# sandialabs/implicit-sph

Measured on AMD Instinct MI355X. Metric: pressure-Poisson solves/sec (3D TGV, 1M particles per GPU, GMRES(50)+block-Jacobi ILU(0), tol 1e-8), higher is better.
Workload: dtype f64; 1 GPU; 3D Taylor-Green vortex, 100^3 particles per GPU, Wendland cut=2h (BASELINE configs[1]), state after one Lagrangian step (mode=advect); rows_per_gpu=1000000, global_rows=1000000, nnz_per_gpu=103845090, solver=FGMRES(50) DGKS tol 1e-8, right prec, precond=bjacobi-ilu0, atom_order=lexicographic, library_row_order=bricks, parallelism=domain bricks 1x1x1, RCCL halo + all-reduce, restarts=1, converged=1

## Files before the change

### implicit-sph_amd/csrc/core.hpp

```cpp
#pragma once
#include "common.hpp"
#include "order.hpp"
#include "sell.hpp"

namespace isph { struct HostStager; }

struct isph_neigh_layout {
  const void *nptr = nullptr;
  const int *nidx = nullptr, *colmap = nullptr;
  const void *order = nullptr;
  int n = -1, is_sorted = 0;
  isph::DevBuf<long long> off;
  isph::DevBuf<int> idx, len, sorted;
  void release() { off.release(); idx.release(); len.release(); sorted.release(); nptr = nullptr; nidx = colmap = nullptr; order = nullptr; n = -1; is_sorted = 0; }
};

struct isph_neigh_map {
  const int *rowsrc = nullptr, *idmap = nullptr, *colmap_key = nullptr;
  const int *colkey = nullptr;
  const void *order = nullptr;
};

struct isph_table_cache {
  int ntypes = -1, kernel = -1, dim = -1;
  std::vector<int> kind;
  std::vector<double> h, cutsq;
  isph::DevBuf<int> dkind;
  isph::DevBuf<double> dh, dcutsq, dhinv, dknorm, dkdnorm;
  void release() { dkind.release(); dh.release(); dcutsq.release(); dhinv.release(); dknorm.release(); dkdnorm.release(); ntypes = -1; }
};

struct isph_ctx {
  int device = 0;
  hipStream_t stream = nullptr;
  bool own_stream = false;
  int rank = 0, nranks = 1;
  ncclComm_t comm = nullptr;
  isph_host_transport host_tr = {nullptr, nullptr, nullptr};
  double *hsend = nullptr, *hrecv = nullptr;
  size_t hsend_cap = 0, hrecv_cap = 0;
  bool profile = false;
  int stat_reorth = 0;
  isph::DevBuf<double> partial;
  isph::DevBuf<double> dscal;
  double *hscal = nullptr;
  size_t hscal_cap = 0;
  isph::DevBuf<double> V, Z, wv, tv, rv, pv, nvec, xext, sendbuf, bdev, xdev;
  isph::DevBuf<float> V32;
  isph::DevBuf<double> vcur;
  isph::DevBuf<double> bint, xint;
  isph::DevBuf<int> imask, imask2;
  std::vector<hipEvent_t> ev;
  std::vector<int> ev_class;
  size_t ev_used = 0;
  std::vector<hipEvent_t> hev;
  size_t hev_used = 0;
  hipEvent_t ev0 = nullptr, ev1 = nullptr;
  hipEvent_t ev_fetch = nullptr;
  std::vector<hipEvent_t> ev_ls;
  hipStream_t comm_stream = nullptr;
  hipEvent_t ev_pack = nullptr, ev_halo = nullptr;
  isph::DevBuf<double> xghost;
  isph::HostStager *stager = nullptr;
  bool neigh_hold = false;
  bool pattern_hold = false;
  isph_neigh_layout neigh_cache[2];
  isph_table_cache tables;
  int ordering = 1;
  isph::OrderBox box;
  isph_neigh_map nmap;
  isph::RowOrderPtr held_order;
  const void *held_key[2] = {nullptr, nullptr};
};

namespace isph {
enum ProfClass { PROF_SPMV = 0, PROF_PREC_APPLY, PROF_MULTI_DOT, PROF_MULTI_AXPY_DOT, PROF_MULTI_AXPY_NORM, PROF_ILU_EXTRACT,
                 PROF_ILU_SCHEDULE, PROF_ILU_FACTOR, PROF_NCLASS };
struct ProfScope {
  isph_ctx *c;
  size_t slot = (size_t)-1;
  ProfScope(isph_ctx *ctx, int cls, hipStream_t st = nullptr) : c(ctx) {
    if (!c || !c->profile || (st && st != c->stream)) return;
    if (c->ev_used + 2 > c->ev.size()) {
      hipEvent_t a = nullptr, b = nullptr;
      if (hipEventCreate(&a) != hipSuccess || hipEventCreate(&b) != hipSuccess) return;
      c->ev.push_back(a); c->ev.push_back(b);
      c->ev_class.push_back(cls);
    }
    slot = c->ev_used;
    c->ev_class[slot / 2] = cls;
    c->ev_used += 2;
    (void)hipEventRecord(c->ev[slot], c->stream);
  }
  ~ProfScope() { end(); }
  void end() {
    if (slot != (size_t)-1) (void)hipEventRecord(c->ev[slot + 1], c->stream);
    slot = (size_t)-1;
  }
};
}

struct isph_halo {
  int npeers = 0;
  std::vector<int> peer, send_ptr, recv_ptr;
  isph::DevBuf<int> send_idx;
  int nsend = 0, nrecv = 0;
  isph::DevBuf<int> list_int, list_bnd;
  int n_int = 0, n_bnd = 0;
};

struct isph_pb_rows;
namespace isph { void pb_rows_destroy(isph_pb_rows *R); }

struct isph_mat {
  isph::Sell S;
  isph_halo halo;
  isph::RowOrderPtr order;
  bool local = false;
  bool aux = false;
  isph_pb_rows *pb = nullptr;
  isph::DevBuf<unsigned> emap;
  long long n_updates = 0;
};
```

### implicit-sph_amd/csrc/gmres_host.hpp

```cpp
#pragma once
#include <algorithm>
#include <cmath>
#include <vector>

namespace isph {

struct GmresCycle {
  int m = 0, j = 0;
  std::vector<double> H, cs, sn, g, y;
  double beta = 0.0, scale = 1.0;

  void reset(int m_) {
    m = m_; j = 0;
    H.assign((size_t)(m + 1) * (size_t)m, 0.0);
    cs.assign((size_t)m, 0.0); sn.assign((size_t)m, 0.0); g.assign((size_t)m + 1, 0.0); y.assign((size_t)m, 0.0);
  }
  void start() {
    std::fill(g.begin(), g.end(), 0.0);
    g[0] = beta;
    j = 0;
  }
  double *column() { return &H[(size_t)j * (size_t)(m + 1)]; }
  double push() {
    double *h = column();
    for (int k = 0; k < j; ++k) {
      const double a = cs[k] * h[k] + sn[k] * h[k + 1];
      h[k + 1] = -sn[k] * h[k] + cs[k] * h[k + 1];
      h[k] = a;
    }
    const double a = h[j], bb = h[j + 1], rr = std::hypot(a, bb);
    cs[j] = rr == 0.0 ? 1.0 : a / rr;
    sn[j] = rr == 0.0 ? 0.0 : bb / rr;
    h[j] = rr;
    h[j + 1] = 0.0;
    g[j + 1] = -sn[j] * g[j];
    g[j] = cs[j] * g[j];
    ++j;
    return std::fabs(g[j]);
  }
  const double *solve() {
    for (int k = j - 1; k >= 0; --k) {
      double s = g[k];
      for (int l = k + 1; l < j; ++l) s -= H[(size_t)l * (size_t)(m + 1) + k] * y[l];
      y[k] = s / H[(size_t)k * (size_t)(m + 1) + k];
    }
    return y.data();
  }
};

template <typename Info>
inline bool gmres_after_update(bool f32, Info &inf, int max_iters, int max_restarts) {
  if (f32 && inf.converged) return true;
  if (inf.converged || inf.iters >= max_iters || inf.restarts >= max_restarts) return false;
  ++inf.restarts;
  return true;
}

template <typename Info>
inline bool gmres_after_residual(bool f32, Info &inf, int max_iters, int max_restarts, double beta, double scale, double tol) {
  if (f32 && inf.converged) {
    if (beta / scale <= tol) return false;
    inf.converged = 0;
    if (inf.iters >= max_iters || inf.restarts >= max_restarts) return false;
    ++inf.restarts;
    ++inf.residual_restarts;
  }
  if (beta == 0.0) { inf.converged = 1; return false; }
  return true;
}

}
```

### implicit-sph_amd/csrc/krylov.hpp

```cpp
#pragma once
#include "common.hpp"

namespace isph {

constexpr int kDotBatch = 16;

template <typename BT> struct BasisVec;
template <> struct BasisVec<double> {
  typedef double2 pair;
  typedef double *__restrict__ out;
};
struct BasisOut32 {
  float *col;
  double *cur;
};
template <> struct BasisVec<float> {
  typedef float2 pair;
  typedef BasisOut32 out;
};
__device__ __forceinline__ bool basis_out_set(const double *o) { return o != nullptr; }
__device__ __forceinline__ bool basis_out_set(const BasisOut32 &o) { return o.col != nullptr; }
__device__ __forceinline__ void basis_put(double *o, long long i, double v) { o[i] = v; }
__device__ __forceinline__ void basis_put(const BasisOut32 &o, long long i, double v) {
  const float r = static_cast<float>(v);
// ... 62 lines not shown
                                                      double *__restrict__ partial) {
  __shared__ double sred[kDotBatch + 1][4];
  const int wave = threadIdx.x >> 6, lane = threadIdx.x & 63;
  const long long stride = (long long)gridDim.x * kBlock;
  const long long i0 = (long long)blockIdx.x * kBlock + threadIdx.x;
  for (int k0 = 0; k0 < nk || k0 == 0; k0 += kDotBatch) {
    const int nb = min(kDotBatch, nk - k0);
    const bool last = k0 + kDotBatch >= nk;
    double acc[kDotBatch];
#pragma unroll
    for (int u = 0; u < kDotBatch; ++u) acc[u] = 0.0;
    double ww = 0.0;
    const BT *__restrict__ vb = V + (long long)k0 * ld;
    long long i = i0;
    if (ROWS == 2) {
      for (; i + stride < n; i += 2 * stride) {
        const double wa = w[i], wb = w[i + stride];
        if (last) ww = fma(wb, wb, fma(wa, wa, ww));
        double va[kDotBatch], vc[kDotBatch];
#pragma unroll
        for (int u = 0; u < kDotBatch; ++u)
          if (u < nb) { va[u] = (double)vb[(long long)u * ld + i]; vc[u] = (double)vb[(long long)u * ld + i + stride]; }
#pragma unroll
        for (int u = 0; u < kDotBatch; ++u)
          if (u < nb) acc[u] = fma(vc[u], wb, fma(va[u], wa, acc[u]));
      }
    }
    for (; i < n; i += stride) {
      const double wi = w[i];
      if (last) ww = fma(wi, wi, ww);
#pragma unroll
      for (int u = 0; u < kDotBatch; ++u)
        if (u < nb) acc[u] = fma((double)vb[(long long)u * ld + i], wi, acc[u]);
    }
#pragma unroll
    for (int u = 0; u < kDotBatch; ++u) {
      if (u < nb) {
        const double s = wave_sum(acc[u]);
        if (lane == 0) sred[u][wave] = s;
      }
    }
    if (last) {
      ww = wave_sum(ww);
      if (lane == 0) sred[kDotBatch][wave] = ww;
    }
    __syncthreads();
    if (threadIdx.x < nb)
      partial[(long long)(k0 + threadIdx.x) * gridDim.x + blockIdx.x] =
          (sred[threadIdx.x][0] + sred[threadIdx.x][1]) + (sred[threadIdx.x][2] + sred[threadIdx.x][3]);
    if (last && threadIdx.x == 0)
      partial[(long long)nk * gridDim.x + blockIdx.x] =
          (sred[kDotBatch][0] + sred[kDotBatch][1]) + (sred[kDotBatch][2] + sred[kDotBatch][3]);
    __syncthreads();
    if (last) break;
  }
}

__global__ __launch_bounds__(kBlock) void k_reduce_partials(int nk, int nblk, const double *__restrict__ partial,
                                                            double *__restrict__ out,
                                                            const double *__restrict__ flag = nullptr) {
  __shared__ double sw[4];
  const int k = blockIdx.x;
  if (k >= nk) return;
  if (flag && *flag == 0.0) {
    if (threadIdx.x == 0) out[k] = 0.0;
    return;
  }
  const double *__restrict__ p = partial + (long long)k * nblk;
  double s0 = 0.0, s1 = 0.0, s2 = 0.0, s3 = 0.0;
  int b = threadIdx.x;
  for (; b + 3 * kBlock < nblk; b += 4 * kBlock) {
    s0 += p[b];
    s1 += p[b + kBlock];
    s2 += p[b + 2 * kBlock];
    s3 += p[b + 3 * kBlock];
  }
  for (; b < nblk; b += kBlock) s0 += p[b];
  double s = wave_sum((s0 + s1) + (s2 + s3));
  if ((threadIdx.x & 63) == 0) sw[threadIdx.x >> 6] = s;
  __syncthreads();
  if (threadIdx.x == 0) out[k] = (sw[0] + sw[1]) + (sw[2] + sw[3]);
}

template <typename BT>
__global__ __launch_bounds__(kBlock) void k_multi_axpy_norm(int n, int nk, const BT *__restrict__ V, long long ld,
                                                            const double *__restrict__ c, double *__restrict__ w,
                                                            double *__restrict__ partial,
                                                            const double *__restrict__ dec_old = nullptr,
                                                            const double *__restrict__ dec_dn = nullptr, int dec_force = 0,
                                                            double *__restrict__ dec_out = nullptr,
                                                            typename BasisVec<BT>::out vnext = {}) {
  __shared__ double sw[4];
  __shared__ double sdec[2];
  const bool next = basis_out_set(vnext);
  bool second = true;
  double wfinal2 = 1.0;
  if (dec_old) {
    if (threadIdx.x == 0) {
      double old2 = *dec_old;
      if (dec_dn) old2 = fmax(old2 - dec_dn[0] * dec_dn[0], 0.0);
      const double ww_new = c[nk];
      const bool sec = dec_force || sqrt(ww_new) < M_SQRT1_2 * sqrt(old2);
      double s2 = 0.0;
      for (int k = 0; k < nk; ++k) s2 += c[k] * c[k];
      sdec[0] = sec ? 1.0 : 0.0;
      sdec[1] = sec ? fmax(ww_new - s2, 0.0) : ww_new;
      if (blockIdx.x == 0) { dec_out[0] = sdec[0]; dec_out[1] = sdec[1]; }
    }
    __syncthreads();
    second = sdec[0] != 0.0;
    wfinal2 = sdec[1];
  }
  if (!second && !next) return;
  double a = 1.0;
  if (next) a *= 1.0 / sqrt(wfinal2);
  double ww = 0.0;
  for (long long i = (long long)blockIdx.x * blockDim.x + threadIdx.x; i < n; i += (long long)gridDim.x * blockDim.x) {
    double s = w[i];
    if (second) {
      for (int k = 0; k < nk; ++k) s = fma(-c[k], (double)V[(long long)k * ld + i], s);
      w[i] = s;
    }
    if (next) basis_put(vnext, i, a * s);
    ww = fma(s, s, ww);
  }
  ww = wave_sum(ww);
  if ((threadIdx.x & 63) == 0) sw[threadIdx.x >> 6] = ww;
  __syncthreads();
  if (threadIdx.x == 0) partial[blockIdx.x] = (sw[0] + sw[1]) + (sw[2] + sw[3]);
}

template <int NK, typename BT = double>
__global__ __launch_bounds__(kBlock) void k_multi_axpy_dot(int n, int nk, const BT *__restrict__ V, long long ld,
                                                           const double *__restrict__ c, double *__restrict__ w,
                                                           double *__restrict__ partial) {
  __shared__ double sred[NK + 1][4];
  __shared__ double sc[NK];
  const int wave = threadIdx.x >> 6, lane = threadIdx.x & 63;
  if (threadIdx.x < NK) sc[threadIdx.x] = threadIdx.x < nk ? c[threadIdx.x] : 0.0;
  __syncthreads();
  double acc[NK];
#pragma unroll
  for (int u = 0; u < NK; ++u) acc[u] = 0.0;
  double ww = 0.0;
  const long long stride = (long long)gridDim.x * kBlock;
  if constexpr (sizeof(BT) == 8) {
    for (long long i = (long long)blockIdx.x * kBlock + threadIdx.x; i < n; i += stride) {
      double v[NK];
#pragma unroll
      for (int u = 0; u < NK; ++u) v[u] = u < nk ? V[(long long)u * ld + i] : 0.0;
      double s = w[i];
#pragma unroll
      for (int u = 0; u < NK; ++u) s = fma(-sc[u], v[u], s);
      w[i] = s;
      ww = fma(s, s, ww);
#pragma unroll
      for (int u = 0; u < NK; ++u) acc[u] = fma(v[u], s, acc[u]);
    }
  } else {
    typedef typename BasisVec<BT>::pair pair;
    const long long np = n >> 1;
    double2 *__restrict__ w2 = reinterpret_cast<double2 *>(w);
    for (long long p = (long long)blockIdx.x * kBlock + threadIdx.x; p < np; p += stride) {
      pair v[NK];
#pragma unroll
      for (int u = 0; u < NK; ++u) {
        if (u < nk) v[u] = reinterpret_cast<const pair *>(V + (long long)u * ld)[p];
        else v[u].x = v[u].y = 0;
      }
      double2 s = w2[p];
#pragma unroll
      for (int u = 0; u < NK; ++u) {
        s.x = fma(-sc[u], (double)v[u].x, s.x);
        s.y = fma(-sc[u], (double)v[u].y, s.y);
      }
      w2[p] = s;
      ww = fma(s.y, s.y, fma(s.x, s.x, ww));
#pragma unroll
      for (int u = 0; u < NK; ++u) asm volatile("" : "+v"(v[u].x), "+v"(v[u].y));
#pragma unroll
      for (int u = 0; u < NK; ++u) acc[u] = fma((double)v[u].y, s.y, fma((double)v[u].x, s.x, acc[u]));
    }
    if ((n & 1) && blockIdx.x == 0 && threadIdx.x == 0) {
      const long long i = n - 1;
      double s = w[i];
#pragma unroll
      for (int u = 0; u < NK; ++u)
        if (u < nk) s = fma(-sc[u], (double)V[(long long)u * ld + i], s);
      w[i] = s;
      ww = fma(s, s, ww);
#pragma unroll
      for (int u = 0; u < NK; ++u)
        if (u < nk) acc[u] = fma((double)V[(long long)u * ld + i], s, acc[u]);
    }
  }
#pragma unroll
  for (int u = 0; u < NK; ++u) {
    if (u < nk) {
      const double r = wave_sum(acc[u]);
      if (lane == 0) sred[u][wave] = r;
    }
  }
  ww = wave_sum(ww);
  if (lane == 0) sred[NK][wave] = ww;
// ... 108 lines not shown
```

### implicit-sph_amd/csrc/solver.hpp

```cpp
#pragma once
#include <cmath>
#include <type_traits>

#include "comm.hpp"
#include "core.hpp"
#include "gmres_host.hpp"
#include "krylov.hpp"

namespace isph {

inline int prec_apply_dev(isph_ctx *ctx, const isph_prec *M, const double *r, double *z);
inline int prec_apply_multi_dev(isph_ctx *ctx, const isph_prec *M, int K, const double *const *rs, double *const *zs);

inline int allreduce_inplace(isph_ctx *ctx, double *d, int count) {
  return comm_allreduce(ctx, d, count,  0, ctx->stream);
}

enum { SC_DOT = 0 , SC_Y = 64 , SC_MISC = 128, SC_COUNT = 160 };

constexpr int kMaxLockstep = 4;

inline int ensure_scalars(isph_ctx *ctx) {
  ISPH_CHECK(ctx->dscal.reserve(SC_COUNT * kMaxLockstep));
  ISPH_CHECK(ctx->partial.reserve((size_t)kMaxRedBlocks * 66));
  if (ctx->hscal_cap < (size_t)SC_COUNT * kMaxLockstep) {
    if (ctx->hscal) (void)hipHostFree(ctx->hscal);
    ISPH_CHECK_HIP(hipHostMalloc((void **)&ctx->hscal, (size_t)SC_COUNT * kMaxLockstep * sizeof(double)));
    ctx->hscal_cap = (size_t)SC_COUNT * kMaxLockstep;
  }
  return ISPH_SUCCESS;
}

inline int fetch_scalars(isph_ctx *ctx, int first, int count) {
  ISPH_CHECK_HIP(hipMemcpyAsync(ctx->hscal + first, ctx->dscal.p + first, sizeof(double) * (size_t)count,
                                hipMemcpyDeviceToHost, ctx->stream));
  ISPH_CHECK_HIP(hipStreamSynchronize(ctx->stream));
  return ISPH_SUCCESS;
}

__global__ void k_gather(int n, const int *__restrict__ idx, const double *__restrict__ x, double *__restrict__ out) {
  for (int i = blockIdx.x * blockDim.x + threadIdx.x; i < n; i += gridDim.x * blockDim.x) out[i] = x[idx[i]];
}
__global__ void k_gather_widen(int n, const int *__restrict__ idx, const float *__restrict__ x, double *__restrict__ out) {
  for (int i = blockIdx.x * blockDim.x + threadIdx.x; i < n; i += gridDim.x * blockDim.x) out[i] = (double)x[idx[i]];
}
inline void halo_pack(isph_ctx *ctx, const isph_halo &H, const double *x) {
  hipLaunchKernelGGL(k_gather, dim3(stream_grid(H.nsend)), dim3(kBlock), 0, ctx->stream, H.nsend, H.send_idx.p, x,
                     ctx->sendbuf.p);
}
inline void halo_pack(isph_ctx *ctx, const isph_halo &H, const float *x) {
  hipLaunchKernelGGL(k_gather_widen, dim3(stream_grid(H.nsend)), dim3(kBlock), 0, ctx->stream, H.nsend, H.send_idx.p, x,
                     ctx->sendbuf.p);
}

template <class XT>
inline int halo_begin(isph_ctx *ctx, const isph_mat *A, const XT *x, hipEvent_t *hev = nullptr) {
  ISPH_REQUIRE(comm_active(ctx) && ctx->comm_stream,
               "a matrix with a halo needs a context made by isph_ctx_create_dist or isph_ctx_create_hostcomm");
  const Sell &S = A->S;
  const isph_halo &H = A->halo;
  ISPH_REQUIRE(H.nrecv == S.ncol - S.nrow, "matrix has ghost columns but no matching halo plan");
  ISPH_REQUIRE(H.n_int + H.n_bnd == S.nslices, "halo plan without the interior/boundary slice lists");
  ISPH_CHECK(ctx->xghost.reserve((size_t)(H.nrecv > 0 ? H.nrecv : 1)));
  ISPH_CHECK(ctx->sendbuf.reserve((size_t)(H.nsend > 0 ? H.nsend : 1)));
  if (H.nsend > 0) halo_pack(ctx, H, x);
  ISPH_CHECK_HIP(hipEventRecord(ctx->ev_pack, ctx->stream));
  if (hev) ISPH_CHECK_HIP(hipEventRecord(hev[0], ctx->stream));
  ISPH_CHECK_HIP(hipStreamWaitEvent(ctx->comm_stream, ctx->ev_pack, 0));
  ISPH_CHECK(comm_exchange(ctx, H, ctx->sendbuf.p, ctx->xghost.p, 1, false, ctx->comm_stream));
  ISPH_CHECK_HIP(hipEventRecord(ctx->ev_halo, ctx->comm_stream));
  if (hev) ISPH_CHECK_HIP(hipEventRecord(hev[1], ctx->comm_stream));
  return ISPH_SUCCESS;
}

inline bool sell_cols16(isph_ctx *ctx, const Sell &S) {
  if (S.c16_state != 0) return S.c16_state > 0;
  S.c16_state = -1;
  if (S.nslices == 0 || S.stored == 0) return false;
  DevTmp<int> flag;
  if (flag.reserve(1) != ISPH_SUCCESS || S.col16.reserve((size_t)S.stored) != ISPH_SUCCESS ||
      S.wtab.reserve((size_t)S.nslices * 64) != ISPH_SUCCESS) { flag.release(); return false; }
  int h = 0;
  if (hipMemsetAsync(flag.p, 0, sizeof(int), ctx->stream) == hipSuccess) {
    hipLaunchKernelGGL(k_sell_compress_cols, dim3((S.nslices + 3) / 4), dim3(kBlock), 0, ctx->stream, 0, S.nslices,
                       (const long long *)S.slice_off.p, (const int *)S.col.p, S.col16.p, S.wtab.p, flag.p);
    if (hipMemcpyAsync(&h, flag.p, sizeof(int), hipMemcpyDeviceToHost, ctx->stream) == hipSuccess &&
        hipStreamSynchronize(ctx->stream) == hipSuccess && hipGetLastError() == hipSuccess && h == 0)
      S.c16_state = 1;
  }
  flag.release();
  if (S.c16_state < 0) { S.col16.release(); S.wtab.release(); }
  return S.c16_state > 0;
}

template <bool DOT, bool LIST, bool GHOST>
inline void spmv_launch(isph_ctx *ctx, const Sell &S, bool c16, int nsl, const int *list, const double *x, const double *xg,
                        double *y, const double *nvec, const double *badd = nullptr, double alpha = 1.0,
                        const float *val32 = nullptr) {
  if (nsl <= 0) return;
  int nbp = 0;
  const int grid = spmv_grid(nsl, &nbp);
  double *part = DOT ? ctx->partial.p : nullptr;
  if (val32 && c16)
    hipLaunchKernelGGL((k_sell_spmv16<8, false, LIST, GHOST, float>), dim3(grid), dim3(kBlock), 0, ctx->stream, S.nrow, nsl, nbp,
                       S.slice_off.p, S.col16.p, S.wtab.p, val32, x, y, nvec, part, list, xg, badd, alpha);
  else if (val32)
    hipLaunchKernelGGL((k_sell_spmv<8, false, true, LIST, GHOST, float>), dim3(grid), dim3(kBlock), 0, ctx->stream, S.nrow, nsl, nbp,
                       S.slice_off.p, S.col.p, val32, x, y, nvec, part, list, xg, badd, alpha);
  else if (c16)
    hipLaunchKernelGGL((k_sell_spmv16<8, DOT, LIST, GHOST>), dim3(grid), dim3(kBlock), 0, ctx->stream, S.nrow, nsl, nbp,
// ... 125 lines not shown
    if (c16) {
      if (K == 2) ISPH_SPMM_AXPB(true, 2, S.col16.p, S.wtab.p);
      else if (K == 3) ISPH_SPMM_AXPB(true, 3, S.col16.p, S.wtab.p);
      else ISPH_SPMM_AXPB(true, 4, S.col16.p, S.wtab.p);
    } else {
      if (K == 2) ISPH_SPMM_AXPB(false, 2, S.col.p, nullptr);
      else if (K == 3) ISPH_SPMM_AXPB(false, 3, S.col.p, nullptr);
      else ISPH_SPMM_AXPB(false, 4, S.col.p, nullptr);
    }
  }
#undef ISPH_SPMM_AXPB
  prof.end();
  ISPH_CHECK_HIP(hipGetLastError());
  return ISPH_SUCCESS;
}

struct LinOp {
  isph_ctx *ctx;
  const isph_mat *A;
  const isph_prec *M;
  const double *nvec;
  int n;
  int dim = 1, nloc = 0;
  const isph_mat *const *blk = nullptr;
  double *tmp = nullptr;
  int apply(const double *x, double *y) const {
    if (blk) {
      for (int i = 0; i < dim; ++i) {
        double *yi = y + (size_t)i * nloc;
        bool first = true;
        for (int j = 0; j < dim; ++j) {
          const isph_mat *B = blk[i * dim + j];
          if (!B) continue;
          ISPH_CHECK(spmv_dev(ctx, B, x + (size_t)j * nloc, first ? yi : tmp, nullptr));
          if (!first)
            hipLaunchKernelGGL(k_axpy_dev, dim3(stream_grid(nloc)), dim3(kBlock), 0, ctx->stream, nloc, 1.0,
                               (const double *)nullptr, (const double *)tmp, yi);
          first = false;
        }
        if (first) ISPH_CHECK_HIP(hipMemsetAsync(yi, 0, sizeof(double) * (size_t)nloc, ctx->stream));
      }
      return ISPH_SUCCESS;
    }
    ISPH_CHECK(spmv_dev(ctx, A, x, y, nvec));
    if (nvec)
      hipLaunchKernelGGL(k_axpy_dev, dim3(stream_grid(n)), dim3(kBlock), 0, ctx->stream, n, -1.0,
                         ctx->dscal.p + SC_MISC, nvec, y);
    return ISPH_SUCCESS;
  }
  int prec(const double *r, double *z) const {
    if (!M) {
      ISPH_CHECK_HIP(hipMemcpyAsync(z, r, sizeof(double) * (size_t)n, hipMemcpyDeviceToDevice, ctx->stream));
      return ISPH_SUCCESS;
    }
    if (blk) {
      const double *rs[4];
      double *zs[4];
      for (int i = 0; i < dim && i < 4; ++i) { rs[i] = r + (size_t)i * nloc; zs[i] = z + (size_t)i * nloc; }
      return prec_apply_multi_dev(ctx, M, dim, rs, zs);
    }
    return prec_apply_dev(ctx, M, r, z);
  }
};

inline int dot_dev(isph_ctx *ctx, int n, const double *a, const double *b, const double *c, const double *d, int slot) {
  const int g = stream_grid(n);
  hipLaunchKernelGGL(k_dot2, dim3(g), dim3(kBlock), 0, ctx->stream, n, a, b, c, d, ctx->partial.p);
  hipLaunchKernelGGL(k_reduce_partials, dim3(2), dim3(kBlock), 0, ctx->stream, 2, g, ctx->partial.p, ctx->dscal.p + slot);
  return allreduce_inplace(ctx, ctx->dscal.p + slot, 2);
}

inline int norm_host(isph_ctx *ctx, int n, const double *v, double *out) {
  ISPH_CHECK(dot_dev(ctx, n, v, v, nullptr, nullptr, SC_MISC + 4));
  ISPH_CHECK(fetch_scalars(ctx, SC_MISC + 4, 1));
  *out = std::sqrt(ctx->hscal[SC_MISC + 4]);
  return ISPH_SUCCESS;
}

inline int residual_norm(isph_ctx *ctx, int n, const double *b, double *w, double *out) {
  hipLaunchKernelGGL(k_residual, dim3(stream_grid(n)), dim3(kBlock), 0, ctx->stream, n, b, w);
  return norm_host(ctx, n, w, out);
}

inline int upload_y(isph_ctx *ctx, GmresCycle &c, int mb = 0) {
  std::copy_n(c.solve(), c.j, ctx->hscal + mb + SC_Y);
  ISPH_CHECK_HIP(hipMemcpyAsync(ctx->dscal.p + mb + SC_Y, ctx->hscal + mb + SC_Y, sizeof(double) * (size_t)c.j, hipMemcpyHostToDevice, ctx->stream));
  return ISPH_SUCCESS;
}

inline int project_dev(isph_ctx *ctx, int n, const double *nvec, double *v) {
  ISPH_CHECK(dot_dev(ctx, n, v, nvec, nullptr, nullptr, SC_MISC + 2));
  hipLaunchKernelGGL(k_axpy_dev, dim3(stream_grid(n)), dim3(kBlock), 0, ctx->stream, n, -1.0, ctx->dscal.p + SC_MISC + 2,
                     nvec, v);
  return ISPH_SUCCESS;
}

inline int cgs_pass(isph_ctx *ctx, int n, int nk, const double *V, long long ld, double *w) {
  int g = stream_grid(n);
  if (g > 1024) g = 1024;
  ISPH_CHECK(ctx->partial.reserve((size_t)(nk + 2) * kMaxRedBlocks > (size_t)kMaxRedBlocks * 66 ? (size_t)(nk + 2) * kMaxRedBlocks : (size_t)kMaxRedBlocks * 66));
  hipLaunchKernelGGL((k_multi_dot<1>), dim3(g), dim3(kBlock), 0, ctx->stream, n, nk, V, ld, w, ctx->partial.p);
  hipLaunchKernelGGL(k_reduce_partials, dim3(nk + 1), dim3(kBlock), 0, ctx->stream, nk + 1, g, ctx->partial.p,
                     ctx->dscal.p + SC_DOT);
  ISPH_CHECK(allreduce_inplace(ctx, ctx->dscal.p + SC_DOT, nk + 1));
  const int g2 = stream_grid(n);
  hipLaunchKernelGGL(k_multi_axpy_norm<double>, dim3(g2), dim3(kBlock), 0, ctx->stream, n, nk, V, ld, ctx->dscal.p + SC_DOT, w,
                     ctx->partial.p);
  hipLaunchKernelGGL(k_reduce_partials, dim3(1), dim3(kBlock), 0, ctx->stream, 1, g2, ctx->partial.p,
                     ctx->dscal.p + SC_DOT + nk + 1);
  ISPH_CHECK(allreduce_inplace(ctx, ctx->dscal.p + SC_DOT + nk + 1, 1));
  ISPH_CHECK_HIP(hipGetLastError());
  return fetch_scalars(ctx, SC_DOT, nk + 2);
}

enum { SC_ORTHO = SC_MISC + 20 };
template <typename BT>
inline int ortho_enqueue(isph_ctx *ctx, int n, int nk, const BT *V, long long ld, double *w, int ortho,
                         typename BasisVec<BT>::out vnext, bool deflate = false, int mb = 0) {
  int g = stream_grid(n);
  if (g > 1024) g = 1024;
  ISPH_CHECK(ctx->partial.reserve((size_t)kMaxRedBlocks * 66));
  hipStream_t st = ctx->stream;
  if (sizeof(BT) == 4)
    ISPH_REQUIRE((reinterpret_cast<uintptr_t>(w) & 15) == 0 && (reinterpret_cast<uintptr_t>(V) & 7) == 0 && ld % 2 == 0,
                 "basis_bits = 32: the Krylov vectors must be 16-byte aligned");
  double *dh1 = ctx->dscal.p + mb + SC_DOT, *dh2 = ctx->dscal.p + mb + SC_Y, *dor = ctx->dscal.p + mb + SC_ORTHO;
  constexpr int dot_grid = 512;
  if (g > dot_grid) g = dot_grid;
  {
    ProfScope prof(ctx, PROF_MULTI_DOT);
    if ((reinterpret_cast<uintptr_t>(w) & 15) == 0 && (reinterpret_cast<uintptr_t>(V) & 15) == 0)
      hipLaunchKernelGGL(k_multi_dot_v2<BT>, dim3(g), dim3(kBlock), 0, st, n, nk, V, ld, w, ctx->partial.p);
    else
      hipLaunchKernelGGL((k_multi_dot<2, BT>), dim3(g), dim3(kBlock), 0, st, n, nk, V, ld, w, ctx->partial.p);
  }
  hipLaunchKernelGGL(k_reduce_partials, dim3(nk + 1), dim3(kBlock), 0, st, nk + 1, g, ctx->partial.p, dh1,
                     (const double *)nullptr);
  ISPH_CHECK(allreduce_inplace(ctx, dh1, nk + 1));
  {
    ProfScope prof(ctx, PROF_MULTI_AXPY_DOT);
    if (nk <= 16)
      hipLaunchKernelGGL((k_multi_axpy_dot<16, BT>), dim3(g), dim3(kBlock), 0, st, n, nk, V, ld, dh1, w, ctx->partial.p);
    else if (nk <= 32)
      hipLaunchKernelGGL((k_multi_axpy_dot<32, BT>), dim3(g), dim3(kBlock), 0, st, n, nk, V, ld, dh1, w, ctx->partial.p);
    else if (nk <= 48)
      hipLaunchKernelGGL((k_multi_axpy_dot<48, BT>), dim3(g), dim3(kBlock), 0, st, n, nk, V, ld, dh1, w, ctx->partial.p);
    else
      hipLaunchKernelGGL((k_multi_axpy_dot<64, BT>), dim3(g), dim3(kBlock), 0, st, n, nk, V, ld, dh1, w, ctx->partial.p);
  }
  hipLaunchKernelGGL(k_reduce_partials, dim3(nk + 1), dim3(kBlock), 0, st, nk + 1, g, ctx->partial.p, dh2,
                     (const double *)nullptr);
  ISPH_CHECK(allreduce_inplace(ctx, dh2, nk + 1));
  const int g2 = stream_grid(n);
  {
    ProfScope prof(ctx, PROF_MULTI_AXPY_NORM);
    hipLaunchKernelGGL(k_multi_axpy_norm<BT>, dim3(g2), dim3(kBlock), 0, st, n, nk, V, ld, (const double *)dh2, w, ctx->partial.p,
                       (const double *)(dh1 + nk), deflate ? (const double *)dh1 : (const double *)nullptr, ortho == 1 ? 1 : 0,
                       dor, vnext);
  }
  ISPH_CHECK_HIP(hipGetLastError());
  return ISPH_SUCCESS;
}

inline void ortho_collect(isph_ctx *ctx, int nk, double *h, double *wnorm, int mb = 0) {
  const double *hs = ctx->hscal + mb;
  const bool second = hs[SC_ORTHO] != 0.0;
  if (second) ++ctx->stat_reorth;
  for (int k = 0; k < nk; ++k) h[k] = hs[SC_DOT + k] + (second ? hs[SC_Y + k] : 0.0);
  *wnorm = std::sqrt(hs[SC_ORTHO + 1]);
}

inline int orthogonalize(isph_ctx *ctx, int n, int j, const double *V, long long ld, double *w, double *h, int ortho,
                         double *wnorm) {
  const int nk = j + 1;
  for (int k = 0; k < nk; ++k) h[k] = 0.0;
  if (ortho == 2) {
    double nn = 0.0;
    for (int pass = 0; pass < 2; ++pass)
      for (int k = 0; k < nk; ++k) {
        ISPH_CHECK(cgs_pass(ctx, n, 1, V + (long long)k * ld, ld, w));
        h[k] += ctx->hscal[SC_DOT];
        nn = ctx->hscal[SC_DOT + 2];
      }
    *wnorm = std::sqrt(nn);
    return ISPH_SUCCESS;
  }
  ISPH_CHECK(ortho_enqueue<double>(ctx, n, nk, V, ld, w, ortho, nullptr));
  ISPH_CHECK(fetch_scalars(ctx, 0, SC_COUNT));
  ortho_collect(ctx, nk, h, wnorm);
  return ISPH_SUCCESS;
}

inline int basis_bits_of(const isph_solver_params *prm, int *bits) {
  *bits = prm->basis_bits == 0 ? 64 : prm->basis_bits;
  ISPH_REQUIRE(*bits == 64 || *bits == 32, "basis_bits must be 64 (0 means the same) or 32");
  return ISPH_SUCCESS;
}

template <typename BT>
inline int gmres_t(const LinOp &op, const double *b, double *x, const isph_solver_params *prm, isph_solve_info *info) {
  constexpr bool f32 = std::is_same<BT, float>::value;
  isph_ctx *ctx = op.ctx;
  const int n = op.n, m = prm->num_blocks;
  ISPH_REQUIRE(m >= 1 && m <= 62, "Num Blocks must be in [1,62]");
  const long long ld = ((long long)n + 63) / 64 * 64;
  const bool deflate = !f32 && op.nvec != nullptr && !op.blk && prm->ortho != 2;
  if (f32) {
    ctx->V.release();
    ISPH_CHECK(ctx->V32.reserve((size_t)ld * (size_t)(m + 1)));
    ISPH_CHECK(ctx->vcur.reserve((size_t)ld));
  } else {
    ctx->V32.release();
    ctx->vcur.release();
    ISPH_CHECK(ctx->V.reserve((size_t)ld * (size_t)(m + 2)));
  }
  if (prm->flexible) ISPH_CHECK(ctx->Z.reserve((size_t)ld * (size_t)m));
  ISPH_CHECK(ctx->wv.reserve((size_t)ld));
  ISPH_CHECK(ctx->tv.reserve((size_t)ld));
  BT *Vall, *V;
  if constexpr (f32) Vall = V = ctx->V32.p;
  else { Vall = ctx->V.p; V = ctx->V.p + (deflate ? ld : 0); }
  double *Z = ctx->Z.p, *w = ctx->wv.p, *t = ctx->tv.p, *vcur = ctx->vcur.p;
  auto column = [&](int col) -> typename BasisVec<BT>::out {
    if constexpr (f32) return BasisOut32{V + (long long)col * ld, vcur};
    else return V + (long long)col * ld;
  };
  if constexpr (!f32)
    if (deflate)
    ISPH_CHECK_HIP(hipMemcpyAsync(Vall, op.nvec, sizeof(double) * (size_t)n, hipMemcpyDeviceToDevice, ctx->stream));
  GmresCycle c;
  c.reset(m);
  const int sg = stream_grid(n);
  hipStream_t st = ctx->stream;

  ISPH_CHECK(op.apply(x, w));
  ISPH_CHECK(residual_norm(ctx, n, b, w, &c.beta));
  c.scale = c.beta == 0.0 ? 1.0 : c.beta;
  info->iters = 0;
  info->restarts = 0;
  info->residual_restarts = 0;
  info->converged = 0;
  info->rel_res_implicit = c.beta / c.scale;
  if (c.beta / c.scale <= prm->tol) info->converged = 1;

  while (!info->converged && info->iters < prm->max_iters) {
    hipLaunchKernelGGL(k_scale_copy<BT>, dim3(sg), dim3(kBlock), 0, st, n, (const double *)w, column(0), 1.0 / c.beta, (const double *)nullptr, 0);
    c.start();
    auto enqueue_op = [&](int col) -> int {
      const double *zj, *vj;
      if constexpr (f32) vj = vcur;
      else vj = V + (long long)col * ld;
      if (prm->flexible) {
        ISPH_CHECK(op.prec(vj, Z + (long long)col * ld));
        zj = Z + (long long)col * ld;
      } else {
        ISPH_CHECK(op.prec(vj, t));
        zj = t;
      }
      return deflate ? spmv_dev(ctx, op.A, zj, w, nullptr) : op.apply(zj, w);
    };
    bool op_queued = false;
    while (c.j < m) {
      const int j = c.j;
      if (!op_queued) ISPH_CHECK(enqueue_op(j));
      op_queued = false;
      double *h = c.column();
      double wn = 0.0;
      if (prm->ortho == 2) {
        if constexpr (!f32) {
          ISPH_CHECK(orthogonalize(ctx, n, j, V, ld, w, h, prm->ortho, &wn));
          if (wn != 0.0)
            hipLaunchKernelGGL(k_scale_copy<double>, dim3(sg), dim3(kBlock), 0, st, n, w, V + (long long)(j + 1) * ld, 1.0 / wn,
                               (const double *)nullptr, 0);
        }
      } else {
        const int nkt = j + 1 + (deflate ? 1 : 0);
        ISPH_CHECK(ortho_enqueue<BT>(ctx, n, nkt, Vall, ld, w, prm->ortho, column(j + 1), deflate));
        ISPH_CHECK_HIP(hipMemcpyAsync(ctx->hscal, ctx->dscal.p, sizeof(double) * SC_COUNT, hipMemcpyDeviceToHost, st));
        ISPH_CHECK_HIP(hipEventRecord(ctx->ev_fetch, st));
        if (j + 1 < m && info->iters + 1 < prm->max_iters) {
          ISPH_CHECK(enqueue_op(j + 1));
          op_queued = true;
        }
        ISPH_CHECK_HIP(hipEventSynchronize(ctx->ev_fetch));
        if (deflate) {
          double hh[66];
          ortho_collect(ctx, nkt, hh, &wn);
          for (int k = 0; k <= j; ++k) h[k] = hh[k + 1];
        } else {
          ortho_collect(ctx, nkt, h, &wn);
        }
      }
      h[j + 1] = wn;
      ++info->iters;
      info->rel_res_implicit = c.push() / c.scale;
      if (prm->verbose && ctx->rank == 0 && info->iters % 10 == 0)
        printf(">> isph::gmres iter %d  rel res %.3e\n", info->iters, info->rel_res_implicit);
      if (info->rel_res_implicit <= prm->tol) { info->converged = 1; break; }
      if (info->iters >= prm->max_iters) break;
    }
    const int j = c.j;
    ISPH_CHECK(upload_y(ctx, c));
    if (prm->flexible) {
      hipLaunchKernelGGL(k_multi_axpy<double>, dim3(sg), dim3(kBlock), 0, st, n, j, Z, ld, ctx->dscal.p + SC_Y, x);
    } else {
      hipLaunchKernelGGL(k_fill, dim3(sg), dim3(kBlock), 0, st, n, w, 0.0);
      hipLaunchKernelGGL(k_multi_axpy<BT>, dim3(sg), dim3(kBlock), 0, st, n, j, (const BT *)V, ld, (const double *)(ctx->dscal.p + SC_Y), w);
      ISPH_CHECK(op.prec(w, t));
      hipLaunchKernelGGL(k_axpy_dev, dim3(sg), dim3(kBlock), 0, st, n, 1.0, (const double *)nullptr, t, x);
    }
    ISPH_CHECK_HIP(hipStreamSynchronize(st));
    if (!gmres_after_update(f32, *info, prm->max_iters, prm->max_restarts)) break;
    ISPH_CHECK(op.apply(x, w));
    ISPH_CHECK(residual_norm(ctx, n, b, w, &c.beta));
    if (!gmres_after_residual(f32, *info, prm->max_iters, prm->max_restarts, c.beta, c.scale, prm->tol)) break;
  }
  ISPH_CHECK_HIP(hipGetLastError());
  return ISPH_SUCCESS;
}

inline int gmres(const LinOp &op, const double *b, double *x, const isph_solver_params *prm, isph_solve_info *info) {
  int bits = 64;
  ISPH_CHECK(basis_bits_of(prm, &bits));
  if (bits == 64) return gmres_t<double>(op, b, x, prm, info);
  ISPH_REQUIRE(prm->ortho != 2, "basis_bits = 32 takes DGKS or ICGS: IMGS (ortho = 2) keeps the fp64 basis");
  ISPH_REQUIRE(!op.blk, "basis_bits = 32 is not available for the blocked operator (isph_solve_block)");
  return gmres_t<float>(op, b, x, prm, info);
}

inline bool gmres_lockstep_ok(const LinOp &op, const isph_solver_params *prm, int K) {
  return K >= 2 && K <= kMaxLockstep && !op.nvec && !op.blk && prm->flexible && prm->ortho != 2 && prm->solver_type == 0;
}

template <typename BT>
inline int gmres_lockstep_t(const LinOp &op, int K, const double *const *bs, double *const *xs, const isph_solver_params *prm,
                            isph_solve_info *infos) {
  constexpr bool f32 = std::is_same<BT, float>::value;
  isph_ctx *ctx = op.ctx;
  const int n = op.n, m = prm->num_blocks;
  ISPH_REQUIRE(m >= 1 && m <= 62, "Num Blocks must be in [1,62]");
  const long long ld = ((long long)n + 63) / 64 * 64;
  if (f32) {
    ctx->V.release();
    ISPH_CHECK(ctx->V32.reserve((size_t)ld * (size_t)(m + 1) * (size_t)K));
    ISPH_CHECK(ctx->vcur.reserve((size_t)ld * (size_t)K));
  } else {
    ctx->V32.release();
    ctx->vcur.release();
    ISPH_CHECK(ctx->V.reserve((size_t)ld * (size_t)(m + 2) * (size_t)K));
  }
  ISPH_CHECK(ctx->Z.reserve((size_t)ld * (size_t)m * (size_t)K));
  ISPH_CHECK(ctx->wv.reserve((size_t)ld * (size_t)K));
  while ((int)ctx->ev_ls.size() < K) {
    hipEvent_t e;
    ISPH_CHECK_HIP(hipEventCreateWithFlags(&e, hipEventDisableTiming));
    ctx->ev_ls.push_back(e);
  }
  struct Sys {
    BT *V;
    double *Z, *w, *vcur = nullptr;
    GmresCycle c;
    bool in_cycle = false, done = false;
  };
  std::vector<Sys> sys((size_t)K);
  const int sg = stream_grid(n);
  hipStream_t st = ctx->stream;
  const double *xin[kMaxLockstep];
  double *yout[kMaxLockstep];
  for (int k = 0; k < K; ++k) {
    Sys &s = sys[(size_t)k];
    if constexpr (f32) { s.V = ctx->V32.p + (size_t)k * ld * (size_t)(m + 1); s.vcur = ctx->vcur.p + (size_t)k * ld; }
    else s.V = ctx->V.p + (size_t)k * ld * (size_t)(m + 2);
    s.Z = ctx->Z.p + (size_t)k * ld * (size_t)m;
    s.w = ctx->wv.p + (size_t)k * ld;
    s.c.reset(m);
    infos[k].iters = 0; infos[k].restarts = 0; infos[k].residual_restarts = 0; infos[k].converged = 0;
    xin[k] = xs[k]; yout[k] = s.w;
  }
  ISPH_CHECK(spmm_dev(ctx, op.A, K, xin, yout));
  for (int k = 0; k < K; ++k) {
    Sys &s = sys[(size_t)k];
    ISPH_CHECK(residual_norm(ctx, n, bs[k], s.w, &s.c.beta));
    s.c.scale = s.c.beta == 0.0 ? 1.0 : s.c.beta;
    infos[k].rel_res_implicit = s.c.beta / s.c.scale;
    if (s.c.beta / s.c.scale <= prm->tol) { infos[k].converged = 1; s.done = true; }
  }
  auto column = [&](Sys &s, int col) -> typename BasisVec<BT>::out {
    if constexpr (f32) return BasisOut32{s.V + (long long)col * ld, s.vcur};
    else return s.V + (long long)col * ld;
  };
  auto start_cycle = [&](int k) {
    Sys &s = sys[(size_t)k];
    hipLaunchKernelGGL(k_scale_copy<BT>, dim3(sg), dim3(kBlock), 0, st, n, (const double *)s.w, column(s, 0), 1.0 / s.c.beta, (const double *)nullptr, 0);
    s.c.start();
    s.in_cycle = true;
  };
  auto end_cycle = [&](int k) -> int {
    Sys &s = sys[(size_t)k];
// ... 137 lines not shown
```

Before: 26.00 solves/s (1M-particle bricks; x n_gpus under weak scaling).

## Add mapped-memory mailbox for GMRES scalars, speculative lookahead gating, zero-x0 shortcut

The kernel now writes the orthogonalization coefficients and a sequence number straight into coherent mapped host memory, and the host spin-polls that slot instead of issuing a device-to-host copy and waiting on an event. This removes per-iteration copy and event latency on a single rank. The lookahead operator enqueue is skipped when the extrapolated residual predicts convergence, which avoids a wasted SpMV and preconditioner apply on the final iteration. An initial zero guess is detected with a small kernel so the first operator apply can be replaced by a memset, and w writes are dropped when w is not needed. In exchange it adds host spinning, a timeout fallback path and an extra sync for the zero check.

```diff
diff --git a/implicit-sph_amd/csrc/core.hpp b/implicit-sph_amd/csrc/core.hpp
--- a/implicit-sph_amd/csrc/core.hpp
+++ b/implicit-sph_amd/csrc/core.hpp
@@ -44,7 +44,10 @@
   isph::DevBuf<double> partial;
   isph::DevBuf<double> dscal;
   double *hscal = nullptr;
+  double *hscal_dev = nullptr;
   size_t hscal_cap = 0;
+  unsigned long long gs_seq = 0;
+  unsigned krylov_legacy = 0;
   isph::DevBuf<double> V, Z, wv, tv, rv, pv, nvec, xext, sendbuf, bdev, xdev;
   isph::DevBuf<float> V32;
   isph::DevBuf<double> vcur;
diff --git a/implicit-sph_amd/csrc/gmres_host.hpp b/implicit-sph_amd/csrc/gmres_host.hpp
--- a/implicit-sph_amd/csrc/gmres_host.hpp
+++ b/implicit-sph_amd/csrc/gmres_host.hpp
@@ -48,6 +48,13 @@
   }
 };
 
+constexpr double kSpeculateMargin = 10.0;
+inline bool gmres_speculate(int nhist, double r1, double r2, double tol) {
+  if (nhist < 2 || !(tol > 0.0) || !(r2 > 0.0) || !(r1 > 0.0) || !std::isfinite(r1) || !std::isfinite(r2)) return true;
+  const double next = r1 * (r1 / r2);
+  return !(next <= kSpeculateMargin * tol);
+}
+
 template <typename Info>
 inline bool gmres_after_update(bool f32, Info &inf, int max_iters, int max_restarts) {
   if (f32 && inf.converged) return true;
diff --git a/implicit-sph_amd/csrc/krylov.hpp b/implicit-sph_amd/csrc/krylov.hpp
--- a/implicit-sph_amd/csrc/krylov.hpp
+++ b/implicit-sph_amd/csrc/krylov.hpp
@@ -168,6 +168,13 @@
   if (threadIdx.x == 0) out[k] = (sw[0] + sw[1]) + (sw[2] + sw[3]);
 }
 
+struct HostBox {
+  double *c1 = nullptr, *c2 = nullptr, *dec = nullptr;
+  const double *dc1 = nullptr;
+  unsigned long long *seq_slot = nullptr;
+  unsigned long long seq = 0;
+};
+
 template <typename BT>
 __global__ __launch_bounds__(kBlock) void k_multi_axpy_norm(int n, int nk, const BT *__restrict__ V, long long ld,
                                                             const double *__restrict__ c, double *__restrict__ w,
@@ -175,7 +182,8 @@
                                                             const double *__restrict__ dec_old = nullptr,
                                                             const double *__restrict__ dec_dn = nullptr, int dec_force = 0,
                                                             double *__restrict__ dec_out = nullptr,
-                                                            typename BasisVec<BT>::out vnext = {}) {
+                                                            typename BasisVec<BT>::out vnext = {}, HostBox box = {},
+                                                            int w_dead = 0) {
   __shared__ double sw[4];
   __shared__ double sdec[2];
   const bool next = basis_out_set(vnext);
@@ -196,16 +204,26 @@
     __syncthreads();
     second = sdec[0] != 0.0;
     wfinal2 = sdec[1];
+    if (box.seq_slot && blockIdx.x == 0 && threadIdx.x < kWave) {
+      for (int k = threadIdx.x; k <= nk; k += kWave) {
+        box.c1[k] = box.dc1[k];
+        box.c2[k] = c[k];
+      }
+      if (threadIdx.x == 0) { box.dec[0] = sdec[0]; box.dec[1] = sdec[1]; }
+      __threadfence_system();
+      if (threadIdx.x == 0) __hip_atomic_store(box.seq_slot, box.seq, __ATOMIC_RELEASE, __HIP_MEMORY_SCOPE_SYSTEM);
+    }
   }
   if (!second && !next) return;
   double a = 1.0;
   if (next) a *= 1.0 / sqrt(wfinal2);
   double ww = 0.0;
+  const bool keep_w = !(next && w_dead);
   for (long long i = (long long)blockIdx.x * blockDim.x + threadIdx.x; i < n; i += (long long)gridDim.x * blockDim.x) {
     double s = w[i];
     if (second) {
       for (int k = 0; k < nk; ++k) s = fma(-c[k], (double)V[(long long)k * ld + i], s);
-      w[i] = s;
+      if (keep_w) w[i] = s;
     }
     if (next) basis_put(vnext, i, a * s);
     ww = fma(s, s, ww);
diff --git a/implicit-sph_amd/csrc/solver.hpp b/implicit-sph_amd/csrc/solver.hpp
--- a/implicit-sph_amd/csrc/solver.hpp
+++ b/implicit-sph_amd/csrc/solver.hpp
@@ -1,5 +1,8 @@
 #pragma once
+#include <chrono>
 #include <cmath>
+#include <cstdlib>
+#include <cstring>
 #include <type_traits>
 
 #include "comm.hpp"
@@ -19,13 +22,37 @@
 enum { SC_DOT = 0 , SC_Y = 64 , SC_MISC = 128, SC_COUNT = 160 };
 
 constexpr int kMaxLockstep = 4;
+
+enum KrylovLegacy : unsigned {
+  KL_MAILBOX = 1,
+  KL_SPECULATE = 2,
+  KL_X0 = 4,
+  KL_ALL = 7
+};
+inline unsigned krylov_legacy_env() {
+  const char *e = getenv("ISPH_KRYLOV_LEGACY");
+  if (!e || !e[0] || (e[0] == '0' && !e[1])) return 0;
+  if (e[0] == '1' && !e[1]) return KL_ALL;
+  unsigned bits = 0;
+  for (; *e; ++e) {
+    const int ch = *e | 0x20;
+    if (ch >= 'b' && ch <= 'd') bits |= 1u << (ch - 'b');
+  }
+  return bits;
+}
+
+constexpr size_t kSeqSlot = (size_t)SC_COUNT * kMaxLockstep;
 
 inline int ensure_scalars(isph_ctx *ctx) {
   ISPH_CHECK(ctx->dscal.reserve(SC_COUNT * kMaxLockstep));
   ISPH_CHECK(ctx->partial.reserve((size_t)kMaxRedBlocks * 66));
   if (ctx->hscal_cap < (size_t)SC_COUNT * kMaxLockstep) {
     if (ctx->hscal) (void)hipHostFree(ctx->hscal);
-    ISPH_CHECK_HIP(hipHostMalloc((void **)&ctx->hscal, (size_t)SC_COUNT * kMaxLockstep * sizeof(double)));
+    else ctx->krylov_legacy = krylov_legacy_env();
+    ISPH_CHECK_HIP(hipHostMalloc((void **)&ctx->hscal, (kSeqSlot + 8) * sizeof(double), hipHostMallocMapped | hipHostMallocCoherent));
+    ISPH_CHECK_HIP(hipHostGetDevicePointer((void **)&ctx->hscal_dev, ctx->hscal, 0));
+    std::memset(ctx->hscal, 0, (kSeqSlot + 8) * sizeof(double));
+    ctx->gs_seq = 0;
     ctx->hscal_cap = (size_t)SC_COUNT * kMaxLockstep;
   }
   return ISPH_SUCCESS;
@@ -317,6 +344,21 @@
   return norm_host(ctx, n, w, out);
 }
 
+__global__ void k_flag_nonzero(int n, const double *__restrict__ v, double *__restrict__ flag) {
+  bool any = false;
+  for (long long i = (long long)blockIdx.x * blockDim.x + threadIdx.x; i < n; i += (long long)gridDim.x * blockDim.x)
+    any |= !(v[i] == 0.0);
+  if (__any(any) && (threadIdx.x & 63) == 0) *flag = 1.0;
+}
+inline int vector_is_zero(isph_ctx *ctx, int n, const double *v, bool *zero) {
+  enum { SLOT = 4 };
+  ctx->hscal[kSeqSlot + SLOT] = 0.0;
+  hipLaunchKernelGGL(k_flag_nonzero, dim3(stream_grid(n)), dim3(kBlock), 0, ctx->stream, n, v, ctx->hscal_dev + kSeqSlot + SLOT);
+  ISPH_CHECK_HIP(hipStreamSynchronize(ctx->stream));
+  *zero = ctx->hscal[kSeqSlot + SLOT] == 0.0;
+  return ISPH_SUCCESS;
+}
+
 inline int upload_y(isph_ctx *ctx, GmresCycle &c, int mb = 0) {
   std::copy_n(c.solve(), c.j, ctx->hscal + mb + SC_Y);
   ISPH_CHECK_HIP(hipMemcpyAsync(ctx->dscal.p + mb + SC_Y, ctx->hscal + mb + SC_Y, sizeof(double) * (size_t)c.j, hipMemcpyHostToDevice, ctx->stream));
@@ -351,7 +393,8 @@
 enum { SC_ORTHO = SC_MISC + 20 };
 template <typename BT>
 inline int ortho_enqueue(isph_ctx *ctx, int n, int nk, const BT *V, long long ld, double *w, int ortho,
-                         typename BasisVec<BT>::out vnext, bool deflate = false, int mb = 0) {
+                         typename BasisVec<BT>::out vnext, bool deflate = false, int mb = 0,
+                         unsigned long long *box_seq = nullptr, bool w_dead = false) {
   int g = stream_grid(n);
   if (g > 1024) g = 1024;
   ISPH_CHECK(ctx->partial.reserve((size_t)kMaxRedBlocks * 66));
@@ -386,14 +429,39 @@
   hipLaunchKernelGGL(k_reduce_partials, dim3(nk + 1), dim3(kBlock), 0, st, nk + 1, g, ctx->partial.p, dh2,
                      (const double *)nullptr);
   ISPH_CHECK(allreduce_inplace(ctx, dh2, nk + 1));
+  HostBox box;
+  if (box_seq) *box_seq = 0;
+  if (box_seq && ctx->nranks == 1 && !(ctx->krylov_legacy & KL_MAILBOX)) {
+    double *hm = ctx->hscal_dev + mb;
+    box.c1 = hm + SC_DOT; box.c2 = hm + SC_Y; box.dec = hm + SC_ORTHO; box.dc1 = dh1;
+    box.seq_slot = reinterpret_cast<unsigned long long *>(ctx->hscal_dev + kSeqSlot);
+    box.seq = *box_seq = ++ctx->gs_seq;
+  }
   const int g2 = stream_grid(n);
   {
     ProfScope prof(ctx, PROF_MULTI_AXPY_NORM);
     hipLaunchKernelGGL(k_multi_axpy_norm<BT>, dim3(g2), dim3(kBlock), 0, st, n, nk, V, ld, (const double *)dh2, w, ctx->partial.p,
                        (const double *)(dh1 + nk), deflate ? (const double *)dh1 : (const double *)nullptr, ortho == 1 ? 1 : 0,
-                       dor, vnext);
+                       dor, vnext, box, w_dead ? 1 : 0);
   }
   ISPH_CHECK_HIP(hipGetLastError());
+  return ISPH_SUCCESS;
+}
+
+constexpr int kMailboxPollMs = 20;
+inline int mailbox_wait(isph_ctx *ctx, unsigned long long seq, int mb = 0) {
+  const unsigned long long *slot = reinterpret_cast<const unsigned long long *>(ctx->hscal + kSeqSlot);
+  const auto t0 = std::chrono::steady_clock::now();
+  for (unsigned spin = 0;; ++spin) {
+    if (__atomic_load_n(slot, __ATOMIC_ACQUIRE) == seq) return ISPH_SUCCESS;
+    if ((spin & 255u) == 255u &&
+        std::chrono::steady_clock::now() - t0 > std::chrono::milliseconds(kMailboxPollMs)) break;
+#if defined(__x86_64__)
+    __builtin_ia32_pause();
+#endif
+  }
+  ISPH_CHECK_HIP(hipStreamSynchronize(ctx->stream));
+  ISPH_CHECK_HIP(hipMemcpy(ctx->hscal + mb, ctx->dscal.p + mb, sizeof(double) * SC_COUNT, hipMemcpyDeviceToHost));
   return ISPH_SUCCESS;
 }
 
@@ -468,7 +536,10 @@
   const int sg = stream_grid(n);
   hipStream_t st = ctx->stream;
 
-  ISPH_CHECK(op.apply(x, w));
+  bool x0_zero = false;
+  if (ctx->nranks == 1 && !op.blk && !(ctx->krylov_legacy & KL_X0)) ISPH_CHECK(vector_is_zero(ctx, n, x, &x0_zero));
+  if (x0_zero) ISPH_CHECK_HIP(hipMemsetAsync(w, 0, sizeof(double) * (size_t)n, st));
+  else ISPH_CHECK(op.apply(x, w));
   ISPH_CHECK(residual_norm(ctx, n, b, w, &c.beta));
   c.scale = c.beta == 0.0 ? 1.0 : c.beta;
   info->iters = 0;
@@ -477,6 +548,9 @@
   info->converged = 0;
   info->rel_res_implicit = c.beta / c.scale;
   if (c.beta / c.scale <= prm->tol) info->converged = 1;
+  int nhist = 1;
+  double res1 = c.beta / c.scale, res2 = 0.0;
+  const bool always_ahead = (ctx->krylov_legacy & KL_SPECULATE) != 0;
 
   while (!info->converged && info->iters < prm->max_iters) {
     hipLaunchKernelGGL(k_scale_copy<BT>, dim3(sg), dim3(kBlock), 0, st, n, (const double *)w, column(0), 1.0 / c.beta, (const double *)nullptr, 0);
@@ -510,14 +584,19 @@
         }
       } else {
         const int nkt = j + 1 + (deflate ? 1 : 0);
-        ISPH_CHECK(ortho_enqueue<BT>(ctx, n, nkt, Vall, ld, w, prm->ortho, column(j + 1), deflate));
-        ISPH_CHECK_HIP(hipMemcpyAsync(ctx->hscal, ctx->dscal.p, sizeof(double) * SC_COUNT, hipMemcpyDeviceToHost, st));
-        ISPH_CHECK_HIP(hipEventRecord(ctx->ev_fetch, st));
-        if (j + 1 < m && info->iters + 1 < prm->max_iters) {
+        unsigned long long seq = 0;
+        ISPH_CHECK(ortho_enqueue<BT>(ctx, n, nkt, Vall, ld, w, prm->ortho, column(j + 1), deflate, 0, &seq, true));
+        if (!seq) {
+          ISPH_CHECK_HIP(hipMemcpyAsync(ctx->hscal, ctx->dscal.p, sizeof(double) * SC_COUNT, hipMemcpyDeviceToHost, st));
+          ISPH_CHECK_HIP(hipEventRecord(ctx->ev_fetch, st));
+        }
+        if (j + 1 < m && info->iters + 1 < prm->max_iters &&
+            (always_ahead || !seq || gmres_speculate(nhist, res1, res2, prm->tol))) {
           ISPH_CHECK(enqueue_op(j + 1));
           op_queued = true;
         }
-        ISPH_CHECK_HIP(hipEventSynchronize(ctx->ev_fetch));
+        if (seq) ISPH_CHECK(mailbox_wait(ctx, seq));
+        else ISPH_CHECK_HIP(hipEventSynchronize(ctx->ev_fetch));
         if (deflate) {
           double hh[66];
           ortho_collect(ctx, nkt, hh, &wn);
@@ -529,6 +608,7 @@
       h[j + 1] = wn;
       ++info->iters;
       info->rel_res_implicit = c.push() / c.scale;
+      res2 = res1; res1 = info->rel_res_implicit; ++nhist;
       if (prm->verbose && ctx->rank == 0 && info->iters % 10 == 0)
         printf(">> isph::gmres iter %d  rel res %.3e\n", info->iters, info->rel_res_implicit);
       if (info->rel_res_implicit <= prm->tol) { info->converged = 1; break; }
@@ -549,6 +629,7 @@
     ISPH_CHECK(op.apply(x, w));
     ISPH_CHECK(residual_norm(ctx, n, b, w, &c.beta));
     if (!gmres_after_residual(f32, *info, prm->max_iters, prm->max_restarts, c.beta, c.scale, prm->tol)) break;
+    res1 = c.beta / c.scale;
   }
   ISPH_CHECK_HIP(hipGetLastError());
   return ISPH_SUCCESS;
```

After: 26.60 solves/s (1M-particle bricks; x n_gpus under weak scaling), median of 6. About the same (+2.3%).
